# PeterCalifano/gtsam_PeterCdev

Hardware: AMD Instinct MI355X
Metric: lm_iterations_per_sec (higher is better)
Workload: dtype f64; 1 GPU; bal1723; ordering=schur_nd, replicas=1, parallelism=replicas1

## Files before the change

gtsam_petercdev_amd/csrc/bigfront.hip:

```cpp
#include <hip/hip_runtime.h>

#include <algorithm>
#include <cstdio>
#include <cstdlib>

#include "gsx_internal.h"
#include "kernels.h"

namespace gsx {
namespace {

typedef double v4d __attribute__((ext_vector_type(4)));
constexpr int T = kTile;
constexpr int kMaxChunk = 192;

#ifdef GSX_STAMP
__device__ unsigned long long g_rstamp[16][8];
#define RST_BEGIN unsigned long long rst0__ = __builtin_amdgcn_s_memtime();
#define RST_ADD(slot)                                                              \
  {                                                                                \
    unsigned long long t__ = __builtin_amdgcn_s_memtime();                         \
    if (lane == 0 && blockIdx.x == 0) g_rstamp[wv][slot] += t__ - rst0__;          \
    rst0__ = t__;                                                                  \
  }
// ... 429 lines not shown
        pt[q] = colj ? xm : pt[q];
        E[q] = colj ? ej : E[q];
        if (j < 15) {
          const double xu = (lj > j) ? xm : 0.0;
          pt = __builtin_amdgcn_mfma_f64_16x16x4f64(-xu, xu, pt, 0, 0, 0);
          E = __builtin_amdgcn_mfma_f64_16x16x4f64(-xu, ej, E, 0, 0, 0);
        }
      }
#else
      tile_potrf16_b4(pt, E, li, lk);
#endif
      __builtin_amdgcn_s_setprio(0);
      double* xd = Xd + (size_t)r * 16 * 17;
#pragma unroll
      for (int q = 0; q < 4; ++q) xd[(4 * q + lk) * 17 + li] = E[q];
      asm volatile("s_waitcnt lgkmcnt(0)" ::: "memory");
      if (lane == 0) __hip_atomic_store(&flagE[r], 1, __ATOMIC_RELEASE, __HIP_MEMORY_SCOPE_WORKGROUP);
      RST_ADD(0)
      if (lk == (li & 3)) {
        const int qd = li >> 2;
        const double l = (qd == 0) ? pt[0] : ((qd == 1) ? pt[1] : ((qd == 2) ? pt[2] : pt[3]));
        ldiag[jb + li] = l;
        dinv[jb + li] = 1.0 / l;
        if (jb + li < fw && !(l > 0)) fail = 1;
      }
#pragma unroll
      for (int q = 0; q < 4; ++q) {
        const int i = 4 * q + lk, c = li;
        if (i > c && jb + i < fw) A[(c0 + jb + c) + (i64)(c0 + jb + i) * n] = E[q];
      }
      store_tile(pt, r);
      if (r > 0) {
        store_tile(last, r - 1);
        if (lane == 0) __hip_atomic_fetch_add(&doneCnt[r - 1], 1, __ATOMIC_RELEASE, __HIP_MEMORY_SCOPE_WORKGROUP);
      }
      RST_ADD(4)
    }
  }
  if (fail) sfail = 1;
  lds_bar();

  for (int c = tid; c < fw; c += NW * 64) X[(c0 + c) + (i64)(c0 + c) * n] = dinv[c];
  for (int kb = wv; kb < nt32; kb += NW) {
    if (fw - kb * T <= 16) continue;
    const double* L10 = t10 + (size_t)kb * 16 * 17;
    const double* X00 = Xd + (size_t)(2 * kb) * 16 * 17;
    const double* X11 = Xd + (size_t)(2 * kb + 1) * 16 * 17;
    const int w1 = min(16, fw - kb * T - 16);
    v4d t1 = {0.0, 0.0, 0.0, 0.0}, t2 = {0.0, 0.0, 0.0, 0.0};
#pragma unroll
    for (int s4 = 0; s4 < 4; ++s4) {
      const double a = (li < w1) ? L10[li * 17 + 4 * s4 + lk] : 0.0;
      t1 = __builtin_amdgcn_mfma_f64_16x16x4f64(a, X00[(4 * s4 + lk) * 17 + li], t1, 0, 0, 0);
    }
#pragma unroll
    for (int s4 = 0; s4 < 4; ++s4)
      t2 = __builtin_amdgcn_mfma_f64_16x16x4f64(-X11[li * 17 + 4 * s4 + lk], t1[s4], t2, 0, 0, 0);
#pragma unroll
    for (int q = 0; q < 4; ++q) {
      const int i = 4 * q + lk;
      if (i < w1) A[(c0 + kb * T + li) + (i64)(c0 + kb * T + 16 + i) * n] = t2[q];
    }
  }
  if (tid == 0) {
    int bad = sfail;
    if (d.parent == kStandaloneFront && c0 + fw == F) {
      int e1, e2;
      (void)frexp(ldiag[fw - 1], &e1);
      if (F >= 2) {
        const double p2 = (fw >= 2) ? ldiag[fw - 2] : A[(F - 2) + (i64)(F - 2) * n];
        (void)frexp(p2, &e2);
        if (!(e2 - e1 < 12)) bad = 1;
      } else if (!(e1 > -12)) {
        bad = 1;
      }
    }
    if (bad) report_failure(status, d.front);
  }
}

struct Quad {
  int li, lk, r0, cq0;
  __device__ __forceinline__ Quad() {
    const int lane = threadIdx.x & 63, wv = threadIdx.x >> 6;
    li = lane & 15;
    lk = lane >> 4;
    r0 = 16 * (wv & 1);
    cq0 = 16 * (wv >> 1);
  }
};

static_assert(kMaxChunk / T == 6, "launch_big_rows dispatches on 1..6 column steps");
constexpr int TS = T * (T + 2);

template <int NK>
__global__ void __launch_bounds__(256) big_rows_kernel(const BigDesc* descs, int c0, int chunk, double* arena) {
  extern __shared__ double dyn[];
  const BigDesc d = descs[blockIdx.y];
  const int n = d.N, F = d.F;
  if (c0 >= F) return;
  const int fw = min(chunk, F - c0), base = c0 + fw;
  const int nrb = (n - base + T - 1) / T;
  if ((int)blockIdx.x >= nrb) return;
  constexpr int nk = NK;
  double* Lb = dyn;
  double(*Tt)[T + 2] = (double(*)[T + 2])(dyn + (size_t)2 * nk * TS);
  double(*Xt)[T + 2] = (double(*)[T + 2])(dyn + (size_t)(2 * nk + 1) * TS);
  double* A = arena + d.off;
  double* X = arena + d.xoff;
  const Quad L;
  const int tid = threadIdx.x, row = L.r0 + L.li;
  const int elo = tid & 31, ehi = tid >> 5;

  double stg[NK][4];
  auto fetch = [&](int kc) {
    const int ck = c0 + kc * T, wk = min(T, fw - kc * T);
#pragma unroll
    for (int q = 0; q < 4; ++q) {
      const int kk = elo, c = ehi + 8 * q;
      double v = 0.0;
      if (c < wk && kk < c) v = A[(ck + kk) + (i64)(ck + c) * n];
      else if (c < wk && kk == c) v = X[(ck + c) + (i64)(ck + c) * n];
      stg[0][q] = v;
    }
#pragma unroll
    for (int t = 1; t < NK; ++t) {
      if (kc + t < nk) {
        const int rr = (kc + t) * T;
#pragma unroll
        for (int q = 0; q < 4; ++q) {
          const int c = elo, kk = ehi + 8 * q;
          stg[t][q] = (rr + c < fw && kk < wk) ? X[(c0 + rr + c) + (i64)(ck + kk) * n] : 0.0;
        }
      }
    }
  };
  auto stash = [&](int kc) {
    double* buf = Lb + (size_t)(kc & 1) * nk * TS;
#pragma unroll
    for (int q = 0; q < 4; ++q) buf[(ehi + 8 * q) * (T + 2) + elo] = stg[0][q];
#pragma unroll
    for (int t = 1; t < NK; ++t) {
      if (kc + t < nk) {
#pragma unroll
        for (int q = 0; q < 4; ++q) buf[(size_t)t * TS + elo * (T + 2) + ehi + 8 * q] = stg[t][q];
      }
    }
  };

  for (int rb = blockIdx.x; rb < nrb; rb += gridDim.x) {
    const int ri = base + T * rb, hi = min(T, n - ri);
    fetch(0);
    v4d tk[NK];
#pragma unroll
    for (int k = 0; k < NK; ++k) {
      const int wk = min(T, fw - k * T);
#pragma unroll
      for (int q = 0; q < 4; ++q) {
        const int c = L.cq0 + 4 * q + L.lk;
        tk[k][q] = (row < hi && c < wk) ? A[(ri + row) + (i64)(c0 + k * T + c) * n] : 0.0;
      }
    }
    lds_bar();
    stash(0);
#pragma unroll
    for (int k = 0; k < NK; ++k) {
      const int wk = min(T, fw - k * T);
      const double* buf = Lb + (size_t)(k & 1) * nk * TS;
      if (k + 1 < nk) fetch(k + 1);
#pragma unroll
      for (int q = 0; q < 4; ++q) Tt[row][L.cq0 + 4 * q + L.lk] = tk[k][q];
      lds_bar();
      v4d x = {0.0, 0.0, 0.0, 0.0};
      {
        const double* pa = buf + (L.cq0 + L.li) * (T + 2) + L.lk;
#pragma unroll
        for (int s = 0; s < 8; ++s)
          if (s < 4 || L.cq0 != 0) x = __builtin_amdgcn_mfma_f64_16x16x4f64(pa[4 * s], Tt[row][4 * s + L.lk], x, 0, 0, 0);
      }
#pragma unroll
      for (int q = 0; q < 4; ++q) {
        const int cc = L.cq0 + 4 * q + L.lk;
        Xt[row][cc] = x[q];
        if (row < hi && cc < wk) X[(ri + row) + (i64)(c0 + k * T + cc) * n] = x[q];
      }
      lds_bar();
#pragma unroll
      for (int k2 = k + 1; k2 < NK; ++k2) {
        const double* pa = buf + (size_t)(k2 - k) * TS + (L.cq0 + L.li) * (T + 2) + L.lk;
#pragma unroll
        for (int s = 0; s < 8; ++s)
          tk[k2] = __builtin_amdgcn_mfma_f64_16x16x4f64(-pa[4 * s], Xt[row][4 * s + L.lk], tk[k2], 0, 0, 0);
      }
      if (k + 1 < nk) stash(k + 1);
    }
  }
}

__global__ void __launch_bounds__(256) big_schur_kernel(const BigDesc* descs, int c0, int chunk, double* arena) {
  const BigDesc d = descs[blockIdx.y];
  const int n = d.N, F = d.F;
  if (c0 >= F) return;
  const int fw = min(chunk, F - c0), base = c0 + fw;
  const int ntile = (n - base + T - 1) / T;
  const int t = blockIdx.x;
  if (t >= ntile * (ntile + 1) / 2) return;
  int i = (int)((sqrtf(8.0f * t + 1.0f) - 1.0f) * 0.5f);
  while ((i + 1) * (i + 2) / 2 <= t) ++i;
  while (i * (i + 1) / 2 > t) --i;
  const int j = t - i * (i + 1) / 2;
  const int ri = base + i * T, rj = base + j * T;
  const int hi = min(T, n - ri), hj = min(T, n - rj);
  double* A = arena + d.off;
  const double* X = arena + d.xoff;
  const Quad L;
  const int row = L.r0 + L.li;
  double cv[4];
  bool live[4];
#pragma unroll
  for (int q = 0; q < 4; ++q) {
    const int c = L.cq0 + 4 * q + L.lk;
    live[q] = row < hi && c < hj && !(i == j && row < c);
    cv[q] = live[q] ? A[(ri + row) + (i64)(rj + c) * n] : 0.0;
  }
  const bool ain = L.cq0 + L.li < hj, bin = row < hi;
  const double* pa = X + (rj + L.cq0 + L.li) + (i64)(c0 + L.lk) * n;
  const double* pb = X + (ri + row) + (i64)(c0 + L.lk) * n;
  v4d acc = {0.0, 0.0, 0.0, 0.0};
  {
    constexpr int kSteps = kMaxChunk / 4;
    double a[kSteps], b[kSteps];
#pragma unroll
    for (int s = 0; s < kSteps; ++s) {
      const bool in = 4 * s + L.lk < fw;
      a[s] = (ain && in) ? pa[(i64)(4 * s) * n] : 0.0;
      b[s] = (bin && in) ? pb[(i64)(4 * s) * n] : 0.0;
    }
#pragma unroll
    for (int s = 0; s < kSteps; ++s)
      if (4 * s < fw) acc = __builtin_amdgcn_mfma_f64_16x16x4f64(a[s], b[s], acc, 0, 0, 0);
  }
#pragma unroll
  for (int q = 0; q < 4; ++q)
    if (live[q]) A[(ri + row) + (i64)(rj + L.cq0 + 4 * q + L.lk) * n] = cv[q] - acc[q];
}

}

#ifdef GSX_STAMP
void big_stamp_dump(const char* what) {
  unsigned long long h[16];
  hipDeviceSynchronize();
  hipMemcpyFromSymbol(h, HIP_SYMBOL(g_bstamp), sizeof(h));
  printf("[bstamp] %s: diag prologue %llu | column setup %llu | D %llu | bar1 %llu | O %llu | store %llu | bar2 %llu | U %llu | "
         "inverse %llu  (cycles, wave 0 of block 0)\n", what, h[0], h[1], h[2], h[3], h[4], h[5], h[6], h[7], h[8]);

  unsigned long long z[16] = {0};
  hipMemcpyToSymbol(HIP_SYMBOL(g_bstamp), z, sizeof(z));
  unsigned long long rs[16][8];
  hipMemcpyFromSymbol(rs, HIP_SYMBOL(g_rstamp), sizeof(rs));
  for (int w = 0; w < 12; ++w)
    printf("[rstamp] wave %2d: D %8llu | wait buffer %8llu | wait E %8llu | O+publish %8llu | store %8llu | wait rows %8llu | U %8llu | top %8llu\n",
           w, rs[w][0], rs[w][1], rs[w][2], rs[w][3], rs[w][4], rs[w][5], rs[w][6], rs[w][7]);
  unsigned long long rz[16][8] = {};
  hipMemcpyToSymbol(HIP_SYMBOL(g_rstamp), rz, sizeof(rz));
}
#endif

void plan_big_group(const BigDesc* descs, int count, BigPlan& plan) {
  plan = BigPlan();
  int maxF = 0;
  for (int k = 0; k < count; ++k) maxF = std::max(maxF, descs[k].F);
  if (count == 0 || maxF == 0) return;
  const int nch = (maxF + kMaxChunk - 1) / kMaxChunk;
  plan.chunk = std::min(kMaxChunk, (((maxF + nch - 1) / nch + T - 1) / T) * T);
  for (int c0 = 0; c0 < maxF; c0 += plan.chunk) {
    int fw = 0, rb = 0, pairs = 0;
    for (int k = 0; k < count; ++k) {
      if (descs[k].F <= c0) continue;
      const int w = std::min(plan.chunk, descs[k].F - c0);
      const int nt = (descs[k].N - (c0 + w) + T - 1) / T;
      fw = std::max(fw, w);
      rb = std::max(rb, nt);
      pairs = std::max(pairs, nt * (nt + 1) / 2);
    }
    plan.fw.push_back(fw);
    plan.rb.push_back(rb);
    plan.pairs.push_back(pairs);
  }
}

void launch_big_diag(const BigDesc* descs, int count, const BigPlan& plan, int round, double* arena, DevStatus* status,
                     hipStream_t st) {
  if (!count) return;
  static bool attr = false;
  const auto lds_for = [](int fw) {
    return (size_t)(((fw + T - 1) / T) * T * (T + 1) + ((fw + 15) / 16) * 16 * 17) * sizeof(double);
  };
  const int kTilesLds = (int)lds_for(kMaxChunk);
  if (!attr) {
    hipFuncSetAttribute((const void*)big_diag_kernel<12, 7>, hipFuncAttributeMaxDynamicSharedMemorySize, kTilesLds);
    hipFuncSetAttribute((const void*)big_diag_kernel<12, 5>, hipFuncAttributeMaxDynamicSharedMemorySize, kTilesLds);
    hipFuncSetAttribute((const void*)big_diag_kernel<8, 5>, hipFuncAttributeMaxDynamicSharedMemorySize, kTilesLds);
    hipFuncSetAttribute((const void*)big_diag_kernel<8, 3>, hipFuncAttributeMaxDynamicSharedMemorySize, kTilesLds);
    hipFuncSetAttribute((const void*)big_diag_kernel<4, 3>, hipFuncAttributeMaxDynamicSharedMemorySize, kTilesLds);
    attr = true;
  }
  const int c0 = round * plan.chunk, fw = plan.fw[round];
  const size_t lds = lds_for(fw);
  const int nt16 = (fw + 15) / 16;
  static const bool v1 = std::getenv("GSX_DIAG_V1") != nullptr;
  if (!v1) {
    static bool attr2 = false;
    const auto lds2_for = [](int w) { return (size_t)(((w + 15) / 16) * 16 * 17 + ((w + T - 1) / T) * 16 * 17) * sizeof(double); };
    if (!attr2) {
      hipFuncSetAttribute((const void*)big_diag_rows_kernel<12>, hipFuncAttributeMaxDynamicSharedMemorySize, (int)lds2_for(kMaxChunk));
      hipFuncSetAttribute((const void*)big_diag_rows_kernel<8>, hipFuncAttributeMaxDynamicSharedMemorySize, (int)lds2_for(kMaxChunk));
      hipFuncSetAttribute((const void*)big_diag_rows_kernel<4>, hipFuncAttributeMaxDynamicSharedMemorySize, (int)lds2_for(kMaxChunk));
      attr2 = true;
    }
    const size_t lds2 = lds2_for(fw);
    if (nt16 <= 4) big_diag_rows_kernel<4><<<count, 256, lds2, st>>>(descs, c0, plan.chunk, arena, status);
    else if (nt16 <= 8) big_diag_rows_kernel<8><<<count, 512, lds2, st>>>(descs, c0, plan.chunk, arena, status);
    else big_diag_rows_kernel<12><<<count, 768, lds2, st>>>(descs, c0, plan.chunk, arena, status);
    return;
  }
  if (nt16 <= 4) big_diag_kernel<4, 3><<<count, 256, lds, st>>>(descs, c0, plan.chunk, arena, status);
  else if (nt16 <= 6) big_diag_kernel<8, 3><<<count, 512, lds, st>>>(descs, c0, plan.chunk, arena, status);
  else if (nt16 <= 8) big_diag_kernel<8, 5><<<count, 512, lds, st>>>(descs, c0, plan.chunk, arena, status);
  else if (nt16 <= 10) big_diag_kernel<12, 5><<<count, 768, lds, st>>>(descs, c0, plan.chunk, arena, status);
  else big_diag_kernel<12, 7><<<count, 768, lds, st>>>(descs, c0, plan.chunk, arena, status);
}

template <int NK>
static void launch_rows_nk(const BigDesc* descs, int count, int gx, int c0, int chunk, double* arena, hipStream_t st) {
  static bool attr = false;
  constexpr size_t lds = (size_t)(2 * NK + 2) * TS * sizeof(double);
  if (!attr) {
    hipFuncSetAttribute((const void*)big_rows_kernel<NK>, hipFuncAttributeMaxDynamicSharedMemorySize, (int)lds);
    attr = true;
  }
  big_rows_kernel<NK><<<dim3(gx, count), 256, lds, st>>>(descs, c0, chunk, arena);
}

void launch_big_rows(const BigDesc* descs, int count, const BigPlan& plan, int round, double* arena, hipStream_t st) {
  if (!count || plan.rb[round] <= 0) return;
  int gx = plan.rb[round];
  if ((long)gx * count > 1024) gx = std::max(1, std::min(gx, 1024 / count));
  const int c0 = round * plan.chunk;
  switch ((plan.fw[round] + T - 1) / T) {
    case 1: launch_rows_nk<1>(descs, count, gx, c0, plan.chunk, arena, st); break;
    case 2: launch_rows_nk<2>(descs, count, gx, c0, plan.chunk, arena, st); break;
    case 3: launch_rows_nk<3>(descs, count, gx, c0, plan.chunk, arena, st); break;
    case 4: launch_rows_nk<4>(descs, count, gx, c0, plan.chunk, arena, st); break;
    case 5: launch_rows_nk<5>(descs, count, gx, c0, plan.chunk, arena, st); break;
    default: launch_rows_nk<6>(descs, count, gx, c0, plan.chunk, arena, st); break;
  }
}

void launch_big_schur(const BigDesc* descs, int count, const BigPlan& plan, int round, double* arena, hipStream_t st) {
  if (!count || plan.pairs[round] <= 0) return;
  big_schur_kernel<<<dim3(plan.pairs[round], count), 256, 0, st>>>(descs, round * plan.chunk, plan.chunk, arena);
}

namespace {
constexpr int kBsThreads = 1024;
constexpr int kBsMaxSep = 320;
__global__ void __launch_bounds__(kBsThreads) backsolve_big_kernel(DevSymbolic S, const int* ids, const double* arena,
                                                                   double* delta, DevStatus* status) {
  extern __shared__ double sm[];
  const int f = ids[blockIdx.x];
  if (wildfire_skip(S, f, threadIdx.x == 0)) return;
  const int n = S.fr_N[f], F = S.fr_F[f];
  const double* A = arena + S.fr_off[f];
  const double* X = A + big_panel_offset(n);
  const int* gi = S.gidx + S.gidx_ptr[f];
  const int tid = threadIdx.x, lane = tid & 63, wave = tid >> 6;
  const int nk = (F + T - 1) / T;
  double* xs = sm;
  double* y = xs + ((n + 1) & ~1);
  double* xp = y + nk * T;
  double* inv = xp + T;
  constexpr int kTri = T * (T + 1) / 2;
  double* low = inv + (size_t)nk * kTri;
  for (int r = F + tid; r < n - 1; r += kBsThreads) xs[r] = delta[gi[r]];
  {
    constexpr int kMaxK = kMaxChunk / T, kMaxLow = kMaxK * (kMaxK - 1) / 2;
    double vi[kMaxK], vl[kMaxLow];
#pragma unroll
    for (int q = 0; q < kMaxK; ++q) {
      const int c = tid & 31, r = tid >> 5;
      const int gr = q * T + r, gc = q * T + c;
      vi[q] = 0.0;
      if (q < nk && r >= c && gr < F) vi[q] = (r > c) ? A[gc + (i64)gr * n] : X[gr + (i64)gr * n];
    }
    int tp = 1, tk = 0;
#pragma unroll
    for (int t = 0; t < kMaxLow; ++t) {
      const int r = tid & 31, c = tid >> 5;
      const int gr = tp * T + r, gc = tk * T + c;
      vl[t] = (t < nk * (nk - 1) / 2 && gr < F) ? X[gr + (i64)gc * n] : 0.0;
      if (++tk == tp) ++tp, tk = 0;
    }
#pragma unroll
    for (int q = 0; q < kMaxK; ++q) {
      const int c = tid & 31, r = tid >> 5;
      if (q < nk && r >= c) inv[(size_t)q * kTri + r * (r + 1) / 2 + c] = vi[q];
    }
#pragma unroll
    for (int t = 0; t < kMaxLow; ++t)
      if (t < nk * (nk - 1) / 2) low[(size_t)t * T * T + (tid & 31) * T + (tid >> 5)] = vl[t];
  }
  __syncthreads();
  {
    constexpr int kRC = kBsMaxSep / 64;
    double xr[kRC];
#pragma unroll
    for (int i = 0; i < kRC; ++i) {
      const int r = F + lane + 64 * i;
      xr[i] = (r < n - 1) ? xs[r] : 0.0;
    }
#pragma unroll
    for (int half = 0; half < 2; ++half) {
      double v[6][kRC], dv[6];
#pragma unroll
      for (int j = 0; j < 6; ++j) {
        const int c = wave + 16 * (6 * half + j);
        const double* col = X + (i64)c * n;
#pragma unroll
        for (int i = 0; i < kRC; ++i) {
          const int r = F + lane + 64 * i;
          v[j][i] = (c < F && r < n - 1) ? col[r] : 0.0;
        }
        dv[j] = (c < F && lane == 0) ? col[n - 1] : 0.0;
      }
#pragma unroll
      for (int j = 0; j < 6; ++j) {
        const int c = wave + 16 * (6 * half + j);
        double acc = 0.0;
// ... 297 lines not shown
}

__global__ void __launch_bounds__(256) backsolve_tree_kernel(DevSymbolic S, BacksolveTreeArgs Q, const double* arena,
                                                             double* delta, DevStatus* status) {
  __shared__ double pool[kBsPool];
  __shared__ int s_f;
  const int tid = threadIdx.x;
  for (;;) {
    if (tid == 0) {
      const int t = atomicAdd(Q.head, 1);
      int f = -1;
      if (t < Q.n_roots) {
        f = Q.roots[t];
      } else if (t < Q.n_tickets) {
        const unsigned long long want = (unsigned long long)Q.epoch << 32;
        const unsigned long long* slot = Q.ready + (t - Q.n_roots);
        int polls = 0;
        for (;;) {
          const unsigned long long v = __hip_atomic_load(slot, __ATOMIC_RELAXED, __HIP_MEMORY_SCOPE_AGENT);
          if ((v >> 32 << 32) == want) {
            f = (int)(v & 0xffffffffu);
            break;
          }
          if (++polls > (1 << 20)) {
            atomicAdd(&status->n_nonfinite, 1);
            f = -2;
            break;
          }
          __builtin_amdgcn_s_sleep(8);
        }
      }
      s_f = f;
    }
    __syncthreads();
    int f = s_f;
    if (f < 0) return;
    while (f >= 0) {
      const int F = S.fr_F[f];
      const bool low = S.fr_N[f] - 2 <= kBsSmallSep;
      if (low && F <= kBsSmallF) backsolve_small_body<true>(S, f, arena, delta, status, pool);
      else if (low && F <= 2 * kBsSmallF) backsolve_small2_body<true>(S, f, arena, delta, status, pool);
      else backsolve_panels_body<true>(S, f, arena, delta, status, pool);
      asm volatile("s_waitcnt vmcnt(0)" ::: "memory");
      __syncthreads();
      const int c0 = Q.child_ptr[f], nc = Q.child_ptr[f + 1] - c0;
      if (nc > 1 && tid < 64) {
        int base = 0;
        if (tid == 0) base = atomicAdd(Q.tail, nc - 1);
        base = __shfl(base, 0, 64);
        for (int k = 1 + tid; k < nc; k += 64)
          __hip_atomic_store(Q.ready + base + k - 1, ((unsigned long long)Q.epoch << 32) | (unsigned)Q.children[c0 + k],
                             __ATOMIC_RELAXED, __HIP_MEMORY_SCOPE_AGENT);
      }
      f = nc > 0 ? Q.children[c0] : -1;
    }
  }
}
}

void launch_backsolve_tree(const DevSymbolic& S, const BacksolveTreeArgs& Q, const double* arena, double* delta,
                           DevStatus* status, hipStream_t st) {
  if (Q.n_tickets <= 0) return;
  const int grid = std::min(Q.n_tickets, 256 * 5);
  backsolve_tree_kernel<<<grid, 256, 0, st>>>(S, Q, arena, delta, status);
}

bool backsolve_small_fits(int max_n, int max_F) { return max_F <= 2 * kBsSmallF && max_n <= kSmallMaxN && max_n - 2 <= kBsSmallSep; }

void launch_backsolve_small(const DevSymbolic& S, const int* ids, int count, int max_F, const double* arena, double* delta,
                            DevStatus* status, hipStream_t st) {
  if (!count) return;
  if (max_F <= kBsSmallF) backsolve_small_kernel<<<count, 256, 0, st>>>(S, ids, arena, delta, status);
  else backsolve_small2_kernel<<<count, 256, 0, st>>>(S, ids, arena, delta, status);
}

size_t backsolve_big_lds(int max_n, int max_F, int max_sep_rows) {
  if (max_sep_rows > kBsMaxSep || max_F > kMaxChunk) return 0;
  const size_t nk = (size_t)(max_F + T - 1) / T;
  const size_t doubles = (((size_t)max_n + 1) & ~(size_t)1) + nk * T + T + nk * (T * (T + 1) / 2) + nk * (nk - 1) / 2 * T * T;
  const size_t bytes = doubles * sizeof(double);
  return bytes <= 160 * 1024 - 256 ? bytes : 0;
}

void launch_backsolve_big(const DevSymbolic& S, const int* ids, int count, int max_n, int max_F, const double* arena,
                          double* delta, DevStatus* status, hipStream_t st) {
  if (!count) return;
  static bool attr = false;
  if (!attr) {
    hipFuncSetAttribute((const void*)backsolve_big_kernel, hipFuncAttributeMaxDynamicSharedMemorySize, 160 * 1024 - 256);
    attr = true;
  }
  backsolve_big_kernel<<<count, kBsThreads, backsolve_big_lds(max_n, max_F, 0), st>>>(S, ids, arena, delta, status);
}

}
```

gtsam_petercdev_amd/csrc/kernels.h:

```cpp
#pragma once
#include <hip/hip_runtime.h>

#include <cstdint>
#include <vector>

#include "../../include/gsx.h"

namespace gsx {

typedef long long i64;

struct FactorRec {
  i64 jac_off;
  int s0, s1;
  int meas_off, noise_off;
  int type_kind;
  int rows_dim;
};
struct DevProblem {
  int n_vars, n_factors;
  const int *var_type, *var_dim, *var_state_off, *var_tan_off;
  const int *f_type, *f_rows, *f_key_ptr, *f_vars, *f_noise_kind, *f_cols;
  const i64 *f_meas_off, *f_noise_off, *f_jac_off;
  const double *meas, *noise;
// ... 107 lines not shown
constexpr int kSensorListShift = TL_RANGE_POSE2_POINT_SENSOR - TL_RANGE_POSE2_POINT;
inline int type_list_of(int t, int vt0, int vt1, long long nmeas) {
  switch (t) {
    case GSX_F_LINEAR: return -1;
    case GSX_F_SFM: return TL_SFM;
    case GSX_F_SFM2: return TL_SFM2;
    case GSX_F_PROJECTION: return nmeas > 7 ? TL_PROJECTION_SENSOR : TL_PROJECTION;
    case GSX_F_BEARINGRANGE: return TL_BEARINGRANGE;
    case GSX_F_BETWEEN: return vt0 == GSX_VAR_POSE2 ? TL_BETWEEN_POSE2 : (vt0 == GSX_VAR_POSE3 ? TL_BETWEEN_POSE3 : TL_GENERIC);
    case GSX_F_RANGE:
      return (vt0 == GSX_VAR_POSE2 ? (vt1 == GSX_VAR_POSE2 ? TL_RANGE_POSE2_POSE : TL_RANGE_POSE2_POINT)
                                   : (vt1 == GSX_VAR_POSE3 ? TL_RANGE_POSE3_POSE : TL_RANGE_POSE3_POINT)) +
             (nmeas > 1 ? kSensorListShift : 0);
    case GSX_F_BEARING: return TL_BEARING;
    case GSX_F_STEREO: return nmeas > 9 ? TL_STEREO_SENSOR : TL_STEREO;
    case GSX_F_SMART_PROJECTION: return TL_SMART;
  }
  return TL_GENERIC;
}
struct SmartDev {
  const int* slot;
  double* cams;
  double* cache;
  double* point;
  int* status;
  int* counters;
  int n;
};
void launch_linearize(const DevProblem& P, const int* const type_lists[kNumTypeLists], const int type_counts[kNumTypeLists],
                      const double* values, double* jac, DevStatus* status, hipStream_t st, const SmartDev* smart = nullptr);
void launch_error(const DevProblem& P, const int* const type_lists[kNumTypeLists], const int type_counts[kNumTypeLists],
                  const double* values, double* partials, int n_partials_cap, double* scalars, int slot, hipStream_t st,
                  const SmartDev* smart = nullptr);
void launch_smart_triangulate(const DevProblem& P, const int* list, int n, const double* values, const SmartDev& S, hipStream_t st);
void launch_smart_linearize(const DevProblem& P, const int* list, int n, const SmartDev& S, double* jac, hipStream_t st);
void launch_smart_error(const DevProblem& P, const int* list, int n, const SmartDev& S, double* partials, int blocks,
                        hipStream_t st);
void launch_linear_error(const DevProblem& P, const double* jac, const double* delta, double* partials,
                         int n_partials_cap, double* scalars, int slice, hipStream_t st);
void launch_lin0(const DevProblem& P, const double* jac, double* partials, int cap, double* scalars, hipStream_t st);
void launch_model_error(const DevProblem& P, const DevSymbolic& S, const int* vars, int nvars, const double* H,
                        const double* delta, const double* damp, double* partials, int cap, double* scalars, hipStream_t st);
void launch_retract(const DevProblem& P, const double* values, const double* delta, double* out, hipStream_t st);
void launch_assemble_h_group(const DevProblem& P, const DevSymbolic& S, const int* vars, int count, int threads,
                             int lds_bytes, bool global, const double* jac, double* H, hipStream_t st);
void launch_assemble_h_star_bundles(const DevProblem& P, const DevSymbolic& S, const int* vars, const int2* bundles,
                                    int count, const double* jac, double* H, hipStream_t st);
void launch_assemble_h_diag_star(const DevProblem& P, const DevSymbolic& S, const int* dvars, int dcount, const int* svars,
                                 const int2* bundles, int scount, const double* jac, double* H, hipStream_t st);
void launch_hessian_diag(const DevProblem& P, const DevSymbolic& S, const double* H, double* diag, hipStream_t st);
void launch_make_damping(int n, const double* hdiag, int diagonal, double mind, double maxd, double* damp,
                         hipStream_t st);
void launch_front_small(const DevProblem& P, const DevSymbolic& S, const int* ids, int count, int max_n,
                        int threads, const double* H, const double* damp, const double* scalars, double* arena,
                        DevStatus* status, hipStream_t st);
struct TreeArgs {
  const int* start;
  int nstart;
  int* cursor;
  int* pending;
  const int *up, *npend;
};
void launch_front_tree(const DevProblem& P, const DevSymbolic& S, const TreeArgs& T, int max_n, int threads, const double* H,
                       const double* damp, const double* scalars, double* arena, DevStatus* status, hipStream_t st);
void launch_front_medium(const DevProblem& P, const DevSymbolic& S, const int* ids, int count, int max_panel, int max_n,
                         const double* H, const double* damp, const double* scalars, double* arena, DevStatus* status,
                         hipStream_t st);
void launch_front_tree_med(const DevProblem& P, const DevSymbolic& S, const TreeArgs& T, size_t lds_bytes, const double* H,
                           const double* damp, const double* scalars, double* arena, DevStatus* status, hipStream_t st);
void launch_big_init(const DevProblem& P, const DevSymbolic& S, const BigDesc* descs, int count, int max_n,
                     int max_nfv, const double* H, const double* damp, const double* scalars, double* arena,
                     hipStream_t st);
struct BigPlan {
  int chunk = 0;
  std::vector<int> fw, rb, pairs;
  int rounds() const { return (int)fw.size(); }
};
void plan_big_group(const BigDesc* host_descs, int count, BigPlan& plan);
void launch_big_diag(const BigDesc* descs, int count, const BigPlan& plan, int round, double* arena, DevStatus* status,
                     hipStream_t st);
#ifdef GSX_STAMP
void big_stamp_dump(const char* what);
#endif
void launch_big_rows(const BigDesc* descs, int count, const BigPlan& plan, int round, double* arena, hipStream_t st);
void launch_big_schur(const BigDesc* descs, int count, const BigPlan& plan, int round, double* arena, hipStream_t st);
void launch_front_leaf(const DevProblem& P, const DevSymbolic& S, const LeafRec* recs, int count, int max_panel, int threads,
                       const double* H, const double* damp, const double* scalars, double* arena, DevStatus* status,
                       hipStream_t st);
void launch_front_star_leaf(const DevSymbolic& S, const StarLeafRec* recs, int count, const int* prow, const double* jac,
                            const double* damp, const double* scalars, double* H, double* arena, DevStatus* status,
                            hipStream_t st);
struct GatherSrc {
  i64 off;
  int d2;
  int ldF;
};
struct GatherSeg {
  i64 dst;
  i64 src;
  int n, ld, dims;
  int slot;
};
struct GatherArgs {
  const GatherSeg* segs;
  const GatherSrc* srcs;
  const i64* gt_dst;
  const int *gt_ld, *gt_dims, *gm_task, *gm_slot, *gm_nslots;
  double* scratch;
};
void launch_big_gather(const GatherArgs& G, int seg0, int nseg, int m0, int nm, double* arena, hipStream_t st);
void launch_backsolve(const DevSymbolic& S, const int* ids, int count, int threads, int max_n, const double* arena,
                      double* delta, DevStatus* status, hipStream_t st);
size_t backsolve_big_lds(int max_n, int max_F, int max_sep_rows);
void launch_backsolve_big(const DevSymbolic& S, const int* ids, int count, int max_n, int max_F, const double* arena,
                          double* delta, DevStatus* status, hipStream_t st);
bool backsolve_small_fits(int max_n, int max_F);
void launch_backsolve_small(const DevSymbolic& S, const int* ids, int count, int max_F, const double* arena, double* delta,
                            DevStatus* status, hipStream_t st);
struct BacksolveTreeArgs {
  const int* roots;
  int n_roots, n_tickets;
  const int *child_ptr, *children;
  unsigned long long* ready;
  int *head, *tail;
  unsigned epoch;
};
void launch_backsolve_tree(const DevSymbolic& S, const BacksolveTreeArgs& Q, const double* arena, double* delta,
                           DevStatus* status, hipStream_t st);
struct WildfireArgs {
  const unsigned char *replaced, *dirty;
  unsigned char* changed;
  const double* old_delta;
  DevStatus* status;
  double threshold;
};
void launch_mark_fronts(const int* ids, int count, unsigned char* flags, hipStream_t st);
void launch_wildfire_post(const DevSymbolic& S, const int* ids, int count, bool wave_per_clique, const WildfireArgs& W,
                          double* delta, hipStream_t st);
void launch_backsolve_leaf(const DevSymbolic& S, const LeafRec* recs, int count, int max_F, const double* arena,
                           double* delta, DevStatus* status, hipStream_t st);
void launch_gradient(const DevProblem& P, const DevSymbolic& S, const double* H, double* g, hipStream_t st);
void launch_ax_sqnorm(const DevProblem& P, const double* jac, const double* x, double* partials, int cap, double* scalars,
                      int slot, hipStream_t st);
void launch_vec_dot(const double* a, const double* b, int64_t n, double* partials, int cap, double* scalars, int slot,
                    hipStream_t st);
void launch_vec_axpby(double* out, double alpha, const double* a, double beta, const double* b, int64_t n, hipStream_t st);
void launch_marginal_path(const DevSymbolic& S, const int* path, int npath, int loc, int dA, int max_n, const double* arena,
                          double* out, double* Y, int64_t n_tan, hipStream_t st);
void launch_joint_cross(const double* Ya, const double* Yb, int64_t n_tan, int dA, int dB, double* out, hipStream_t st);
struct MargItem {
  int front, ti, tj, pad;
};
struct MargArgs {
  const i64 *slot, *work;
  double* cov;
  const double* arena;
  const i64* out_off;
  const int* var_dim;
  double* out;
};
void launch_marg_prep(const DevSymbolic& S, const MargArgs& M, const MargItem* items, int count, hipStream_t st);
void launch_marg_kt(const DevSymbolic& S, const MargArgs& M, const MargItem* items, int count, hipStream_t st);
void launch_marg_sf(const DevSymbolic& S, const MargArgs& M, const MargItem* items, int count, hipStream_t st);
void launch_marg_ff(const DevSymbolic& S, const MargArgs& M, const MargItem* items, int count, hipStream_t st);
void launch_marg_emit(const DevSymbolic& S, const MargArgs& M, const int2* vars, int count, hipStream_t st);
void launch_marg_leaf(const DevSymbolic& S, const MargArgs& M, const int* ids, int count, hipStream_t st);
void launch_set_scalar(double* scalars, int slot, double v, hipStream_t st);
// ... 51 lines not shown
```

gtsam_petercdev_amd/csrc/kernels.hip:

```cpp
#include <hip/hip_runtime.h>

#include <climits>
#include <cstdio>
#include <cstdlib>

#include "device_geometry.h"
#include "gsx_internal.h"
#include "kernels.h"

namespace gsx {
using namespace gsxd;

#define T kTile

__device__ __forceinline__ double wave_sum(double v) {
#pragma unroll
  for (int o = 32; o > 0; o >>= 1) v += __shfl_down(v, o, 64);
  return v;
}
typedef double v4d __attribute__((ext_vector_type(4)));
__device__ __forceinline__ i64 readlane_i64(i64 v, int src_lane) {
  int lo = (int)(v & 0xFFFFFFFFll), hi = (int)(v >> 32);
  lo = __builtin_amdgcn_readlane(lo, src_lane);
  hi = __builtin_amdgcn_readlane(hi, src_lane);
// ... 3243 lines not shown
      for (int q = lane; q < nfv; q += step) W.changed[S.fvars[S.fr_fvar_ptr[f] + q]] = 1;
    } else {
      for (int r = lane; r < F; r += step) {
        const int g = gi[r];
        delta[g] = W.old_delta[g];
      }
    }
  }
  __syncthreads();
  if (threadIdx.x == 0 && solved) atomicAdd(&W.status->n_backsub, solved);
}
void launch_wildfire_post(const DevSymbolic& S, const int* ids, int count, bool wave_per_clique, const WildfireArgs& W,
                          double* delta, hipStream_t st) {
  if (count <= 0) return;
  if (wave_per_clique) wildfire_post_kernel<true><<<(count + 3) / 4, 256, 0, st>>>(S, ids, count, W, delta);
  else wildfire_post_kernel<false><<<(count + 255) / 256, 256, 0, st>>>(S, ids, count, W, delta);
}
__global__ void __launch_bounds__(256) mark_fronts_kernel(const int* ids, int count, unsigned char* flags) {
  const int k = blockIdx.x * blockDim.x + threadIdx.x;
  if (k < count) flags[ids[k]] = 1;
}
void launch_mark_fronts(const int* ids, int count, unsigned char* flags, hipStream_t st) {
  if (count > 0) mark_fronts_kernel<<<(count + 255) / 256, 256, 0, st>>>(ids, count, flags);
}

void launch_backsolve(const DevSymbolic& S, const int* ids, int count, int threads, int max_n, const double* arena,
                      double* delta, DevStatus* status, hipStream_t st) {
  static bool attr = false;
  if (!attr) {
    hipFuncSetAttribute((const void*)backsolve_kernel, hipFuncAttributeMaxDynamicSharedMemorySize, 128 * 1024);
    attr = true;
  }
  if (count)
    backsolve_kernel<<<count, threads, (size_t)max_n * sizeof(double), st>>>(S, ids, arena, delta, status);
}

__global__ void dense_small_kernel(double* a, int n, int nf, DevStatus* status) {
  extern __shared__ double L[];
  __shared__ FrontScratch sc;
  for (int e = threadIdx.x; e < n * n; e += blockDim.x) L[e] = a[e];
  __syncthreads();
  const int fail = lds_partial_cholesky(L, n, nf, true, sc);
  if (fail && threadIdx.x == 0) report_failure(status, 0);
  for (int e = threadIdx.x; e < n * n; e += blockDim.x) {
    const int r = e % n, c = e / n;
    if (r >= c) a[e] = L[e];
  }
}
void launch_dense_partial(double* a, int n, int nf, DevStatus* status, hipStream_t st) {
  if (nf == 0) return;
  if (n <= kSmallMaxN) {
    static bool attr = false;
    if (!attr) {
      hipFuncSetAttribute((const void*)dense_small_kernel, hipFuncAttributeMaxDynamicSharedMemorySize, 160 * 1024 - 4096);
      attr = true;
    }
    dense_small_kernel<<<1, 512, (size_t)n * n * sizeof(double), st>>>(a, n, nf, status);
#ifdef GSX_STAMP
    {
      unsigned long long h[8];
      hipStreamSynchronize(st);
      hipMemcpyFromSymbol(h, HIP_SYMBOL(g_stamp), sizeof(h));
      printf("[stamp] n=%d F=%d panel-factor %llu cycles, trailing %llu cycles\n", n, nf, h[0], h[1]);
      unsigned long long z[8] = {0};
      hipMemcpyToSymbol(HIP_SYMBOL(g_stamp), z, sizeof(z));
    }
#endif
    return;
  }
  double* work = nullptr;
  const i64 xoff = big_panel_offset(n);
  hipMalloc(&work, (size_t)(xoff + (i64)n * nf) * sizeof(double));
  hipMemcpyAsync(work, a, (size_t)n * n * sizeof(double), hipMemcpyDeviceToDevice, st);
  double* const user = a;
  a = work;
  BigDesc h{0, xoff, n, nf, 0, kStandaloneFront};
  BigDesc* d = nullptr;
  hipMalloc(&d, sizeof(BigDesc));
  hipMemcpyAsync(d, &h, sizeof(BigDesc), hipMemcpyHostToDevice, st);
  BigPlan plan;
  plan_big_group(&h, 1, plan);
  for (int r = 0; r < plan.rounds(); ++r) {
    launch_big_diag(d, 1, plan, r, a, status, st);
    launch_big_rows(d, 1, plan, r, a, st);
    launch_big_schur(d, 1, plan, r, a, st);
  }
  big_copy_panel_kernel<<<64, 256, 0, st>>>(d, a);
  hipMemcpyAsync(user, work, (size_t)n * n * sizeof(double), hipMemcpyDeviceToDevice, st);
  hipStreamSynchronize(st);
#ifdef GSX_STAMP
  {
    char what[64];
    snprintf(what, sizeof(what), "n=%d F=%d", n, nf);
    big_stamp_dump(what);
  }
#endif
  hipFree(d);
  hipFree(work);
}

}
```

gtsam_petercdev_amd/csrc/solver.hip:

```cpp
#include <hip/hip_runtime.h>

#include <algorithm>
#include <cstdlib>
#include <chrono>
#include <climits>
#include <cmath>
#include <cstdio>
#include <cstring>
#include <limits>
#include <array>
#include <map>
#include <string>
#include <vector>

#include "gsx_internal.h"
#include "kernels.h"

using namespace gsx;

namespace {

#define HIPCHK(ctx, expr)                                                                  \
  do {                                                                                     \
    hipError_t e__ = (expr);                                                               \
// ... 1147 lines not shown
  if (c->damp_kind != 0) c->damp_ready = false;
  c->solved = false;
}

void dev_assemble_h(gsx_context* c) {
  timer_begin(c, PH_ASSEMBLE_H);
  const gsx_context::HGroup *gs = nullptr, *gd = nullptr;
  for (const auto& g : c->hgroups) {
    if (g.threads == -1 && c->n_star_bundles) gs = &g;
    if (g.threads == 0 && g.count > 0) gd = &g;
  }
  const bool fs = c->fused_star;
  const bool fused = gs && gd && !fs;
  if (fused)
    launch_assemble_h_diag_star(c->DP, c->DS, c->d_hvars.p + gd->begin, gd->count, c->d_hvars.p + gs->begin,
                                c->d_star_bundles.p, c->n_star_bundles, c->d_jac.p, c->d_H.p, c->stream);
  for (const auto& g : c->hgroups) {
    if (fused && (&g == gs || &g == gd)) continue;
    if (fs && g.threads == -1) {
      if (c->n_star_rest)
        launch_assemble_h_group(c->DP, c->DS, c->d_star_rest_vars.p, c->n_star_rest, -1, 0, false, c->d_jac.p, c->d_H.p,
                                c->stream);
      continue;
    }
    if (g.threads == -1 && c->n_star_bundles) {
      launch_assemble_h_star_bundles(c->DP, c->DS, c->d_hvars.p + g.begin, c->d_star_bundles.p, c->n_star_bundles,
                                     c->d_jac.p, c->d_H.p, c->stream);
      continue;
    }
    launch_assemble_h_group(c->DP, c->DS, c->d_hvars.p + g.begin, g.count, g.threads, g.lds, g.global, c->d_jac.p,
                            c->d_H.p, c->stream);
  }
  timer_end(c, PH_ASSEMBLE_H);
  c->h_ready = true;
  c->hstar_ready = !fs;
  c->hdiag_ready = false;
}

void dev_ensure_hstar(gsx_context* c) {
  if (c->hstar_ready) return;
  for (const auto& g : c->hgroups) {
    if (g.threads != -1) continue;
    if (c->n_star_bundles)
      launch_assemble_h_star_bundles(c->DP, c->DS, c->d_hvars.p + g.begin, c->d_star_bundles.p, c->n_star_bundles,
                                     c->d_jac.p, c->d_H.p, c->stream);
    else
      launch_assemble_h_group(c->DP, c->DS, c->d_hvars.p + g.begin, g.count, g.threads, g.lds, g.global, c->d_jac.p,
                              c->d_H.p, c->stream);
  }
  c->hstar_ready = true;
}

void dev_hessian_diag(gsx_context* c) {
  if (c->hdiag_ready) return;
  dev_ensure_hstar(c);
  launch_hessian_diag(c->DP, c->DS, c->d_H.p, c->d_hdiag.p, c->stream);
  if (c->con_hd_n)
    launch_constraint_hdiag(c->con_hd_n, c->d_con_hd_tan.p, c->d_con_hd_ptr.p, c->d_con_hd_jidx.p, c->d_con_hd_w.p,
                            c->d_jac.p, c->d_hdiag.p, c->stream);
  if (c->sharded()) {
    launch_mask_copy(c->d_hdiag.p, c->d_sched_tan.p, c->P.tan_size, c->d_hdiag.p, c->stream);
    shard_allreduce(c, c->d_hdiag.p, c->P.tan_size);
  }
  c->hdiag_ready = true;
}

void dev_damping(gsx_context* c, int diagonal, double mind, double maxd) {
  if (c->damp_ready && c->damp_kind == diagonal && (diagonal == 0 || (c->damp_min == mind && c->damp_max == maxd))) return;
  if (diagonal) dev_hessian_diag(c);
  launch_make_damping((int)c->P.tan_size, c->d_hdiag.p, diagonal, mind, maxd, c->d_damp.p, c->stream);
  if (c->sharded()) launch_mask_copy(c->d_damp.p, c->d_own_tan.p, c->P.tan_size, c->d_damp.p, c->stream);
  c->damp_ready = true;
  c->damp_kind = diagonal;
  c->damp_min = mind;
  c->damp_max = maxd;
}

void dev_big_factor(gsx_context* c, const BigDesc* descs, int count, const BigPlan& plan, hipStream_t st, bool prof) {
  for (int r = 0; r < plan.rounds(); ++r) {
    if (prof) timer_begin(c, PH_K_POTRF0);
    launch_big_diag(descs, count, plan, r, c->d_arena.p, c->d_status.p, st);
    if (prof) timer_end(c, PH_K_POTRF0);
    if (prof) timer_begin(c, PH_K_TRSM);
    launch_big_rows(descs, count, plan, r, c->d_arena.p, st);
    if (prof) timer_end(c, PH_K_TRSM);
    if (prof) timer_begin(c, PH_K_SYRK);
    launch_big_schur(descs, count, plan, r, c->d_arena.p, st);
    if (prof) timer_end(c, PH_K_SYRK);
  }
}

void debug_sync(gsx_context* c, const char* what, int a, int b) {
  static const bool on = std::getenv("GSX_DEBUG_LAUNCH") != nullptr;
  if (!on) return;
  fprintf(stderr, "[gsx] %s (%d, %d) ...", what, a, b);
  fflush(stderr);
  const hipError_t e = hipStreamSynchronize(c->stream);
  const hipError_t e2 = hipGetLastError();
  fprintf(stderr, " %s / %s\n", hipGetErrorString(e), hipGetErrorString(e2));
  fflush(stderr);
}

void dev_leaf_group(gsx_context* c, size_t g, hipStream_t st) {
  const SmallLaunch& sl = c->leaf_launch[0][g];
  if (c->fused_star && c->leaf_split[g].scount) {
    const gsx_context::LeafSplit& ls = c->leaf_split[g];
    launch_front_star_leaf(c->DS, c->d_star_recs.p + ls.sbegin, ls.scount, c->d_star_prow.p, c->d_jac.p, c->d_damp.p,
                           c->d_scalars.p, c->d_H.p, c->d_arena.p, c->d_status.p, st);
    if (ls.rcount)
      launch_front_leaf(c->DP, c->DS, c->d_leaf_rest_recs.p + ls.rbegin, ls.rcount, sl.max_panel, sl.threads, c->d_H.p,
                        c->d_damp.p, c->d_scalars.p, c->d_arena.p, c->d_status.p, st);
    return;
  }
  launch_front_leaf(c->DP, c->DS, c->d_leaf_recs.p + (sl.begin - c->leaf_base), sl.count, sl.max_panel, sl.threads, c->d_H.p,
                    c->d_damp.p, c->d_scalars.p, c->d_arena.p, c->d_status.p, st);
}

bool bulk_ready(gsx_context* c) {
  if (c->bulk) return true;
  int least = 0, greatest = 0;
  if (hipDeviceGetStreamPriorityRange(&least, &greatest) != hipSuccess) return false;
  if (hipStreamCreateWithPriority(&c->bulk, hipStreamNonBlocking, least) != hipSuccess) {
    c->bulk = nullptr;
    return false;
  }
  if (hipEventCreateWithFlags(&c->bulk_go, hipEventDisableTiming) != hipSuccess ||
      hipEventCreateWithFlags(&c->bulk_done, hipEventDisableTiming) != hipSuccess)
    return false;
  return true;
}

void dev_factorize(gsx_context* c, double lambda) {
  const Symbolic& S = c->S;
  c->fact_valid = false;
  c->fact_pending = true;
  c->fact_lambda = lambda;
  c->wf_all_replaced = true;
  c->sc_dirty |= kXFact;
  timer_begin(c, PH_FACTORIZE);
  launch_begin_factorization(c->d_scalars.p, lambda, c->d_status.p, c->d_tree_cursor.p, c->stream);
  if (!c->big_descs.empty())
    launch_big_init(c->DP, c->DS, c->d_big.p, (int)c->big_descs.size(), c->big_max_n, c->big_max_nfv, c->d_H.p,
                    c->d_damp.p, c->d_scalars.p, c->d_arena.p, c->stream);
  const int sg = S.n_ulevels;
  const bool have_side = S.side_level0 >= 0;
  const bool use_bulk = have_side && c->profiling <= 0 && bulk_ready(c);
  if (S.n_levels > 0) {
    const std::vector<SmallLaunch>& LL = c->leaf_launch[0];
    const size_t n_main_leaf = c->leaf_side_group0 != (size_t)-1 ? c->leaf_side_group0 : LL.size();
    if (use_bulk) {
      hipEventRecord(c->bulk_go, c->stream);
      hipStreamWaitEvent(c->bulk, c->bulk_go, 0);
      for (size_t g = n_main_leaf; g < LL.size(); ++g) dev_leaf_group(c, g, c->bulk);
      launch_big_gather(c->GA, S.gseg_lvl_ptr[sg], S.gseg_lvl_ptr[sg + 1] - S.gseg_lvl_ptr[sg], S.gm_lvl_ptr[sg],
                        S.gm_lvl_ptr[sg + 1] - S.gm_lvl_ptr[sg], c->d_arena.p, c->bulk);
      hipEventRecord(c->bulk_done, c->bulk);
      c->bulk_pending = true;
    }
    for (size_t g = 0; g < (use_bulk ? n_main_leaf : LL.size()); ++g) {
      if (c->profiling > 0) timer_begin(c, PH_FACTOR_LEAF);
      dev_leaf_group(c, g, c->stream);
      if (c->profiling > 0) timer_end(c, PH_FACTOR_LEAF);
    }
  }
  for (size_t t = 0; t < c->tree_tiers.size(); ++t) {
    const gsx_context::TreeTier& tt = c->tree_tiers[t];
    if (!tt.nstart) continue;
// ... 2403 lines not shown
```

Baseline: 579.2 LM iterations/s.

## Share staged triangular panel across two row tiles per block in big_rows

When there are more row tiles than CUs, the big_rows TRSM kernel now runs 512-thread blocks that process two 32-row tiles at once. Both halves share one LDS-staged copy of the L panel, and each half keeps its own Tt/Xt scratch. This halves the number of panel loads and stashes per row, and for two halves the first panel fetch is hoisted out of the row loop. In exchange it adds LDS per block, raises register pressure, and leaves fewer blocks when rows are scarce. A refusal path reports failure when the panel does not fit in LDS.

New measurement: 588.4 LM iterations/s, median of 6. 1.02x the previous value.

```diff
diff --git a/gtsam_petercdev_amd/csrc/bigfront.hip b/gtsam_petercdev_amd/csrc/bigfront.hip
--- a/gtsam_petercdev_amd/csrc/bigfront.hip
+++ b/gtsam_petercdev_amd/csrc/bigfront.hip
@@ -535,7 +535,7 @@
 struct Quad {
   int li, lk, r0, cq0;
   __device__ __forceinline__ Quad() {
-    const int lane = threadIdx.x & 63, wv = threadIdx.x >> 6;
+    const int lane = threadIdx.x & 63, wv = (threadIdx.x >> 6) & 3;
     li = lane & 15;
     lk = lane >> 4;
     r0 = 16 * (wv & 1);
@@ -545,32 +545,37 @@
 
 static_assert(kMaxChunk / T == 6, "launch_big_rows dispatches on 1..6 column steps");
 constexpr int TS = T * (T + 2);
-
-template <int NK>
-__global__ void __launch_bounds__(256) big_rows_kernel(const BigDesc* descs, int c0, int chunk, double* arena) {
+constexpr size_t kLdsPerCU = 160 * 1024;
+
+template <int NK, int NH>
+__global__ void __launch_bounds__(256 * NH) big_rows_kernel(const BigDesc* descs, int c0, int chunk, double* arena) {
   extern __shared__ double dyn[];
+  constexpr int RB = T * NH;
+  constexpr int NQ = 4 / NH;
+  constexpr int EH = 8 * NH;
   const BigDesc d = descs[blockIdx.y];
   const int n = d.N, F = d.F;
   if (c0 >= F) return;
   const int fw = min(chunk, F - c0), base = c0 + fw;
-  const int nrb = (n - base + T - 1) / T;
+  const int nrb = (n - base + RB - 1) / RB;
   if ((int)blockIdx.x >= nrb) return;
   constexpr int nk = NK;
+  const int tid = threadIdx.x;
+  const int half = __builtin_amdgcn_readfirstlane(tid >> 8);
   double* Lb = dyn;
-  double(*Tt)[T + 2] = (double(*)[T + 2])(dyn + (size_t)2 * nk * TS);
-  double(*Xt)[T + 2] = (double(*)[T + 2])(dyn + (size_t)(2 * nk + 1) * TS);
+  double(*Tt)[T + 2] = (double(*)[T + 2])(dyn + (size_t)(2 * nk + 2 * half) * TS);
+  double(*Xt)[T + 2] = (double(*)[T + 2])(dyn + (size_t)(2 * nk + 2 * half + 1) * TS);
   double* A = arena + d.off;
   double* X = arena + d.xoff;
   const Quad L;
-  const int tid = threadIdx.x, row = L.r0 + L.li;
+  const int row = L.r0 + L.li;
   const int elo = tid & 31, ehi = tid >> 5;
 
-  double stg[NK][4];
-  auto fetch = [&](int kc) {
+  auto fetch = [&](int kc, double (&stg)[NK][NQ]) {
     const int ck = c0 + kc * T, wk = min(T, fw - kc * T);
 #pragma unroll
-    for (int q = 0; q < 4; ++q) {
-      const int kk = elo, c = ehi + 8 * q;
+    for (int q = 0; q < NQ; ++q) {
+      const int kk = elo, c = ehi + EH * q;
       double v = 0.0;
       if (c < wk && kk < c) v = A[(ck + kk) + (i64)(ck + c) * n];
       else if (c < wk && kk == c) v = X[(ck + c) + (i64)(ck + c) * n];
@@ -581,29 +586,31 @@
       if (kc + t < nk) {
         const int rr = (kc + t) * T;
 #pragma unroll
-        for (int q = 0; q < 4; ++q) {
-          const int c = elo, kk = ehi + 8 * q;
+        for (int q = 0; q < NQ; ++q) {
+          const int c = elo, kk = ehi + EH * q;
           stg[t][q] = (rr + c < fw && kk < wk) ? X[(c0 + rr + c) + (i64)(ck + kk) * n] : 0.0;
         }
       }
     }
   };
-  auto stash = [&](int kc) {
+  auto stash = [&](int kc, const double (&stg)[NK][NQ]) {
     double* buf = Lb + (size_t)(kc & 1) * nk * TS;
 #pragma unroll
-    for (int q = 0; q < 4; ++q) buf[(ehi + 8 * q) * (T + 2) + elo] = stg[0][q];
+    for (int q = 0; q < NQ; ++q) buf[(ehi + EH * q) * (T + 2) + elo] = stg[0][q];
 #pragma unroll
     for (int t = 1; t < NK; ++t) {
       if (kc + t < nk) {
 #pragma unroll
-        for (int q = 0; q < 4; ++q) buf[(size_t)t * TS + elo * (T + 2) + ehi + 8 * q] = stg[t][q];
+        for (int q = 0; q < NQ; ++q) buf[(size_t)t * TS + elo * (T + 2) + ehi + EH * q] = stg[t][q];
       }
     }
   };
 
+  double stg0[NK][NQ], stg[NK][NQ];
+  if constexpr (NH == 2) fetch(0, stg0);
   for (int rb = blockIdx.x; rb < nrb; rb += gridDim.x) {
-    const int ri = base + T * rb, hi = min(T, n - ri);
-    fetch(0);
+    const int ri = base + RB * rb + T * half, hi = min(T, n - ri);
+    if constexpr (NH == 1) fetch(0, stg);
     v4d tk[NK];
 #pragma unroll
     for (int k = 0; k < NK; ++k) {
@@ -615,12 +622,13 @@
       }
     }
     lds_bar();
-    stash(0);
+    if constexpr (NH == 2) stash(0, stg0);
+    else stash(0, stg);
 #pragma unroll
     for (int k = 0; k < NK; ++k) {
       const int wk = min(T, fw - k * T);
       const double* buf = Lb + (size_t)(k & 1) * nk * TS;
-      if (k + 1 < nk) fetch(k + 1);
+      if (k + 1 < nk) fetch(k + 1, stg);
 #pragma unroll
       for (int q = 0; q < 4; ++q) Tt[row][L.cq0 + 4 * q + L.lk] = tk[k][q];
       lds_bar();
@@ -645,7 +653,7 @@
         for (int s = 0; s < 8; ++s)
           tk[k2] = __builtin_amdgcn_mfma_f64_16x16x4f64(-pa[4 * s], Xt[row][4 * s + L.lk], tk[k2], 0, 0, 0);
       }
-      if (k + 1 < nk) stash(k + 1);
+      if (k + 1 < nk) stash(k + 1, stg);
     }
   }
 }
@@ -785,29 +793,69 @@
   else big_diag_kernel<12, 7><<<count, 768, lds, st>>>(descs, c0, plan.chunk, arena, status);
 }
 
+size_t big_rows_lds(int fw, long tiles, int cus, int* rows) {
+  if (fw <= 0 || fw > kMaxChunk || tiles <= 0 || cus <= 0) return 0;
+  const int nk = (fw + T - 1) / T, nh = tiles > cus ? 2 : 1;
+  const size_t bytes = (size_t)(2 * nk + 2 * nh) * TS * sizeof(double);
+  if (bytes > kLdsPerCU) return 0;
+  if (rows) *rows = T * nh;
+  return bytes;
+}
+extern "C" long long gsxtest_big_rows_lds(int fw, long long tiles, int cus, int* rows) {
+  int r = 0;
+  const size_t bytes = big_rows_lds(fw, (long)tiles, cus, &r);
+  if (rows) *rows = bytes ? r : 0;
+  return (long long)bytes;
+}
+
+namespace {
+__global__ void rows_refused_kernel(const BigDesc* descs, DevStatus* status) { report_failure(status, descs[0].front); }
+
+template <int NK, int NH>
+void launch_rows_nk(const BigDesc* descs, int count, int gx, int c0, int chunk, size_t lds, double* arena, hipStream_t st) {
+  static bool attr = false;
+  if (!attr) {
+    hipFuncSetAttribute((const void*)big_rows_kernel<NK, NH>, hipFuncAttributeMaxDynamicSharedMemorySize, (int)lds);
+    attr = true;
+  }
+  big_rows_kernel<NK, NH><<<dim3(gx, count), 256 * NH, lds, st>>>(descs, c0, chunk, arena);
+}
 template <int NK>
-static void launch_rows_nk(const BigDesc* descs, int count, int gx, int c0, int chunk, double* arena, hipStream_t st) {
-  static bool attr = false;
-  constexpr size_t lds = (size_t)(2 * NK + 2) * TS * sizeof(double);
-  if (!attr) {
-    hipFuncSetAttribute((const void*)big_rows_kernel<NK>, hipFuncAttributeMaxDynamicSharedMemorySize, (int)lds);
-    attr = true;
-  }
-  big_rows_kernel<NK><<<dim3(gx, count), 256, lds, st>>>(descs, c0, chunk, arena);
-}
-
-void launch_big_rows(const BigDesc* descs, int count, const BigPlan& plan, int round, double* arena, hipStream_t st) {
+void launch_rows(int rows, const BigDesc* descs, int count, int gx, int c0, int chunk, size_t lds, double* arena,
+                 hipStream_t st) {
+  if (rows == 2 * T) launch_rows_nk<NK, 2>(descs, count, gx, c0, chunk, lds, arena, st);
+  else launch_rows_nk<NK, 1>(descs, count, gx, c0, chunk, lds, arena, st);
+}
+}
+
+void launch_big_rows(const BigDesc* descs, int count, const BigPlan& plan, int round, double* arena, DevStatus* status,
+                     hipStream_t st) {
   if (!count || plan.rb[round] <= 0) return;
-  int gx = plan.rb[round];
+  static int cus = 0;
+  if (!cus) {
+    int dev = 0;
+    if (hipGetDevice(&dev) != hipSuccess ||
+        hipDeviceGetAttribute(&cus, hipDeviceAttributeMultiprocessorCount, dev) != hipSuccess)
+      cus = 0;
+  }
+  int rows = T;
+  const size_t lds = big_rows_lds(plan.fw[round], (long)plan.rb[round] * count, cus, &rows);
+  if (!lds) {
+    fprintf(stderr, "gsx: big_rows cannot stage a chunk of %d columns in LDS (%d CUs): launch refused, the factorization fails\n",
+            plan.fw[round], cus);
+    rows_refused_kernel<<<1, 1, 0, st>>>(descs, status);
+    return;
+  }
+  int gx = (plan.rb[round] * T + rows - 1) / rows;
   if ((long)gx * count > 1024) gx = std::max(1, std::min(gx, 1024 / count));
   const int c0 = round * plan.chunk;
   switch ((plan.fw[round] + T - 1) / T) {
-    case 1: launch_rows_nk<1>(descs, count, gx, c0, plan.chunk, arena, st); break;
-    case 2: launch_rows_nk<2>(descs, count, gx, c0, plan.chunk, arena, st); break;
-    case 3: launch_rows_nk<3>(descs, count, gx, c0, plan.chunk, arena, st); break;
-    case 4: launch_rows_nk<4>(descs, count, gx, c0, plan.chunk, arena, st); break;
-    case 5: launch_rows_nk<5>(descs, count, gx, c0, plan.chunk, arena, st); break;
-    default: launch_rows_nk<6>(descs, count, gx, c0, plan.chunk, arena, st); break;
+    case 1: launch_rows<1>(rows, descs, count, gx, c0, plan.chunk, lds, arena, st); break;
+    case 2: launch_rows<2>(rows, descs, count, gx, c0, plan.chunk, lds, arena, st); break;
+    case 3: launch_rows<3>(rows, descs, count, gx, c0, plan.chunk, lds, arena, st); break;
+    case 4: launch_rows<4>(rows, descs, count, gx, c0, plan.chunk, lds, arena, st); break;
+    case 5: launch_rows<5>(rows, descs, count, gx, c0, plan.chunk, lds, arena, st); break;
+    default: launch_rows<6>(rows, descs, count, gx, c0, plan.chunk, lds, arena, st); break;
   }
 }
 
@@ -1271,6 +1319,10 @@
   return bytes <= 160 * 1024 - 256 ? bytes : 0;
 }
 
+extern "C" long long gsxtest_backsolve_big_lds(int max_n, int max_F, int max_sep_rows) {
+  return (long long)backsolve_big_lds(max_n, max_F, max_sep_rows);
+}
+
 void launch_backsolve_big(const DevSymbolic& S, const int* ids, int count, int max_n, int max_F, const double* arena,
                           double* delta, DevStatus* status, hipStream_t st) {
   if (!count) return;
diff --git a/gtsam_petercdev_amd/csrc/kernels.h b/gtsam_petercdev_amd/csrc/kernels.h
--- a/gtsam_petercdev_amd/csrc/kernels.h
+++ b/gtsam_petercdev_amd/csrc/kernels.h
@@ -213,7 +213,9 @@
 #ifdef GSX_STAMP
 void big_stamp_dump(const char* what);
 #endif
-void launch_big_rows(const BigDesc* descs, int count, const BigPlan& plan, int round, double* arena, hipStream_t st);
+size_t big_rows_lds(int fw, long tiles, int cus, int* rows);
+void launch_big_rows(const BigDesc* descs, int count, const BigPlan& plan, int round, double* arena, DevStatus* status,
+                     hipStream_t st);
 void launch_big_schur(const BigDesc* descs, int count, const BigPlan& plan, int round, double* arena, hipStream_t st);
 void launch_front_leaf(const DevProblem& P, const DevSymbolic& S, const LeafRec* recs, int count, int max_panel, int threads,
                        const double* H, const double* damp, const double* scalars, double* arena, DevStatus* status,
diff --git a/gtsam_petercdev_amd/csrc/kernels.hip b/gtsam_petercdev_amd/csrc/kernels.hip
--- a/gtsam_petercdev_amd/csrc/kernels.hip
+++ b/gtsam_petercdev_amd/csrc/kernels.hip
@@ -3349,7 +3349,7 @@
   plan_big_group(&h, 1, plan);
   for (int r = 0; r < plan.rounds(); ++r) {
     launch_big_diag(d, 1, plan, r, a, status, st);
-    launch_big_rows(d, 1, plan, r, a, st);
+    launch_big_rows(d, 1, plan, r, a, status, st);
     launch_big_schur(d, 1, plan, r, a, st);
   }
   big_copy_panel_kernel<<<64, 256, 0, st>>>(d, a);
diff --git a/gtsam_petercdev_amd/csrc/solver.hip b/gtsam_petercdev_amd/csrc/solver.hip
--- a/gtsam_petercdev_amd/csrc/solver.hip
+++ b/gtsam_petercdev_amd/csrc/solver.hip
@@ -1253,7 +1253,7 @@
     launch_big_diag(descs, count, plan, r, c->d_arena.p, c->d_status.p, st);
     if (prof) timer_end(c, PH_K_POTRF0);
     if (prof) timer_begin(c, PH_K_TRSM);
-    launch_big_rows(descs, count, plan, r, c->d_arena.p, st);
+    launch_big_rows(descs, count, plan, r, c->d_arena.p, c->d_status.p, st);
     if (prof) timer_end(c, PH_K_TRSM);
     if (prof) timer_begin(c, PH_K_SYRK);
     launch_big_schur(descs, count, plan, r, c->d_arena.p, st);
```
